# Pointcept/Pointcept

Measured on AMD Instinct MI355X. Metric: scenes/sec (fwd+bwd+optimizer) PTv3 ScanNet-semseg @ ~100k pts, higher is better.
Workload: dtype bf16; 1 GPU; PT-v3m1 base (46.2M params) + seg head + CE + Lovasz, fwd+bwd+AdamW, 8 scenes x 102400 voxels per GPU, patch 1024, 4 orders; global_batch=8, parallelism=dp1, params=46167572, amp=bf16 autocast, points_per_gpu=819200, loss=CrossEntropy(ignore_index=-1) + LovaszSoftmax

## Files before the change

### pointcept_amd/csrc/gemm3.h

```cpp
#pragma once
#include "ptc_common.h"

int ptc_gemm3_launch(int dtype, const void* in, int64_t n_in, const void* w, const float* bias, const int32_t* nbr, int64_t n_out, int kv, int c_in,
                     int c_out, void* out, hipStream_t s, int epi, const void* aux_in, void* aux_out);
bool ptc_gemm3_supported(int dtype, int kv, int c_in, int c_out);

#ifdef PTC_GEMM3_IMPL
#include "mma.h"

#define G3_BN 128
#define G3_BK 64
#ifndef G3_STAGGER
#define G3_STAGGER 0
#endif

__device__ __forceinline__ int g3_lds_row_of_channel(int n) { return 16 * ((n & 15) >> 2) + 4 * (n >> 4) + (n & 3); }
template <typename T> __device__ __forceinline__ uint32_t g3_pack2(float lo, float hi);
template <> __device__ __forceinline__ uint32_t g3_pack2<bf16_t>(float lo, float hi) { return ptc_pack_bf16x2(lo, hi); }
template <> __device__ __forceinline__ uint32_t g3_pack2<f16_t>(float lo, float hi) {
  const _Float16 a = (_Float16)lo, b = (_Float16)hi;
  return (uint32_t)(*reinterpret_cast<const uint16_t*>(&a)) | ((uint32_t)(*reinterpret_cast<const uint16_t*>(&b)) << 16);
}
template <typename T> __device__ __forceinline__ void g3_store16(T* dst, const float (&v)[16]) {
  uint32_t pk[8];
#pragma unroll
  for (int i = 0; i < 8; ++i) pk[i] = g3_pack2<T>(v[2 * i], v[2 * i + 1]);
  reinterpret_cast<uint4*>(dst)[0] = make_uint4(pk[0], pk[1], pk[2], pk[3]);
  reinterpret_cast<uint4*>(dst)[1] = make_uint4(pk[4], pk[5], pk[6], pk[7]);
}

__device__ __forceinline__ int g3_off(int row, int p) { return row * (G3_BK * 2) + ((p ^ ((row >> 1) & 7)) << 4); }

template <typename T, int EPI, int RS>
__global__ void __launch_bounds__(256) PTC_WAVES_PER_EU(2, 2)
gemm3_kernel(const T* __restrict__ in, const T* __restrict__ w, const float* __restrict__ bias, const int32_t* __restrict__ nbr, int64_t n_out,
             int kv, int c_in, int c_out, T* __restrict__ out, const T* __restrict__ aux_in, T* __restrict__ aux_out, uint32_t in_bytes,
             int n_col_tiles, int n_tiles) {
  using M = Mma<T>;
  constexpr int BM = RS * 32;
  constexpr int A_BYTES = BM * G3_BK * 2, STAGE_BYTES = A_BYTES + G3_BN * G3_BK * 2;
  extern __shared__ __attribute__((aligned(16))) unsigned char smem[];
  const __amdgpu_buffer_rsrc_t in_buf = ptc_buf(in, in_bytes);
  const int lane = ptc_lane(), wave = threadIdx.x >> 6;
  const int r = lane & 15, g = lane >> 4;
  const int wm = wave & 1, wn = wave >> 1;

  const int PX = (int)gridDim.x >> 3, px = (int)blockIdx.x >> 3, xcd = (int)blockIdx.x & 7;
  const int tx0 = (int)((int64_t)n_tiles * xcd / 8), tx1 = (int)((int64_t)n_tiles * (xcd + 1) / 8);
  if (tx0 + px >= tx1) return;
  if (G3_STAGGER > 0 && px >= PX / 2) __builtin_amdgcn_s_sleep(G3_STAGGER);
  const int n_my = (tx1 - tx0 - px + PX - 1) / PX;
  const int cpk = c_in / G3_BK, cpt = kv * cpk, total = n_my * cpt;

  const int kp = threadIdx.x & 7, rr = threadIdx.x >> 3;
  int lds_a[RS], lds_w[4];
#pragma unroll
  for (int i = 0; i < RS; ++i) lds_a[i] = g3_off(rr + 32 * i, kp);
#pragma unroll
  for (int i = 0; i < 4; ++i) {
    const int row = rr + 32 * i;
    lds_w[i] = A_BYTES + g3_off((row & 64) + g3_lds_row_of_channel(row & 63), kp);
  }

  int lj = 0, lk = 0, lc = 0;
  int64_t l_row0 = 0;
  int l_n0 = 0;
  uint32_t a_cur[RS];
  int32_t idx_next[RS];
  const T* w_cur[4];
  f32x4 bias_r[4];
  ptc_i32x4 ra0[RS], rw0[4], ra1[RS], rw1[4];
  auto set_tile = [&]() __attribute__((always_inline)) {
    const int t = tx0 + px + lj * PX;
    const int row_tile = t / n_col_tiles;
    l_row0 = (int64_t)row_tile * BM;
    l_n0 = (t - row_tile * n_col_tiles) * G3_BN;
  };
  auto request_idx = [&](int j, int k) __attribute__((always_inline)) {
    const int t = tx0 + px + j * PX;
    const int64_t row0 = (int64_t)(t / n_col_tiles) * BM;
#pragma unroll
    for (int i = 0; i < RS; ++i) {
      const int64_t row = row0 + rr + 32 * i;
      int32_t v = -1;
      if (row < n_out) v = nbr ? nbr[(int64_t)k * n_out + row] : (int32_t)row;
      idx_next[i] = v;
    }
  };
  auto enter_segment = [&]() __attribute__((always_inline)) {
#pragma unroll
    for (int i = 0; i < RS; ++i)
      a_cur[i] = idx_next[i] >= 0 ? ((uint32_t)idx_next[i] * (uint32_t)c_in + (uint32_t)(kp * 8)) * 2u : PTC_BUF_OOB;
#pragma unroll
    for (int i = 0; i < 4; ++i) w_cur[i] = w + ((int64_t)(l_n0 + rr + 32 * i) * kv + lk) * c_in + kp * 8;
  };
  auto issue_chunk = [&](ptc_i32x4 (&ra)[RS], ptc_i32x4 (&rw)[4]) __attribute__((always_inline)) {
    const int c0 = lc * G3_BK;
#pragma unroll
    for (int i = 0; i < RS; ++i)
      ra[i] = __builtin_amdgcn_raw_buffer_load_b128(in_buf, (int)(a_cur[i] == PTC_BUF_OOB ? PTC_BUF_OOB : a_cur[i] + (uint32_t)c0 * 2u), 0, 0);
#pragma unroll
    for (int i = 0; i < 4; ++i) rw[i] = *reinterpret_cast<const ptc_i32x4*>(w_cur[i] + c0);
  };
  auto request_bias = [&]() __attribute__((always_inline)) {
#pragma unroll
    for (int t = 0; t < 4; ++t) {
      bias_r[t] = (f32x4){0.f, 0.f, 0.f, 0.f};
      if (bias) bias_r[t] = *reinterpret_cast<const f32x4*>(bias + l_n0 + wn * 64 + 16 * g + 4 * t);
    }
  };
  auto request_following = [&]() __attribute__((always_inline)) {
    if (lk + 1 < kv) request_idx(lj, lk + 1);
    else if (lj + 1 < n_my) request_idx(lj + 1, 0);
  };
  auto store_chunk = [&](int st, const ptc_i32x4 (&ra)[RS], const ptc_i32x4 (&rw)[4]) __attribute__((always_inline)) {
    unsigned char* base = smem + st * STAGE_BYTES;
#pragma unroll
    for (int i = 0; i < RS; ++i) *reinterpret_cast<ptc_i32x4*>(base + lds_a[i]) = ra[i];
#pragma unroll
    for (int i = 0; i < 4; ++i) *reinterpret_cast<ptc_i32x4*>(base + lds_w[i]) = rw[i];
  };
  auto advance = [&]() __attribute__((always_inline)) {
    if (++lc == cpk) {
      lc = 0;
      if (++lk == kv) { lk = 0; ++lj; }
    }
  };

  int64_t p_row0 = 0;
  int p_n0 = 0;
  auto fetch = [&](ptc_i32x4 (&ra)[RS], ptc_i32x4 (&rw)[4], bool live) __attribute__((always_inline)) {
    const bool seg_start = live && lc == 0, tile_start = seg_start && lk == 0;
    if (tile_start) { set_tile(); p_row0 = l_row0; p_n0 = l_n0; }
    if (seg_start) enter_segment();
    if (tile_start) request_bias();
    if (seg_start) request_following();
    issue_chunk(ra, rw);
    if (live) advance();
  };

  request_idx(0, 0);
  fetch(ra0, rw0, true);
  int64_t c_row0 = p_row0;
  int c_n0 = p_n0;
  int crem = 0;
  fetch(ra1, rw1, true);
  store_chunk(0, ra0, rw0);
  __syncthreads();

  f32x4 acc[RS][4];
  auto half = [&](int it, ptc_i32x4 (&raL)[RS], ptc_i32x4 (&rwL)[4], const ptc_i32x4 (&raS)[RS], const ptc_i32x4 (&rwS)[4]) __attribute__((always_inline)) {
    if (crem == 0) {
#pragma unroll
      for (int t = 0; t < 4; ++t)
#pragma unroll
        for (int s = 0; s < RS; ++s) acc[s][t] = bias_r[t];
    }
    fetch(raL, rwL, it + 2 < total);
    const unsigned char* As = smem + (it & 1) * STAGE_BYTES;
    const unsigned char* Ws = As + A_BYTES;
#pragma unroll
    for (int ks = 0; ks < G3_BK / 32; ++ks) {
      typename M::frag fw[4], fa[RS];
#pragma unroll
      for (int t = 0; t < 4; ++t) fw[t] = *reinterpret_cast<const typename M::frag*>(Ws + g3_off(wn * 64 + t * 16 + r, ks * 4 + g));
#pragma unroll
      for (int s = 0; s < RS; ++s) fa[s] = *reinterpret_cast<const typename M::frag*>(As + g3_off(wm * (RS * 16) + s * 16 + r, ks * 4 + g));
#pragma unroll
      for (int s = 0; s < RS; ++s)
#pragma unroll
        for (int t = 0; t < 4; ++t) acc[s][t] = M::mma(fw[t], fa[s], acc[s][t]);
    }
    if (crem == cpt - 1) {
#pragma unroll
      for (int s = 0; s < RS; ++s) {
        const int64_t row = c_row0 + wm * (RS * 16) + s * 16 + r;
        if (row >= n_out) continue;
        const int64_t off = row * c_out + c_n0 + wn * 64 + 16 * g;
        float v[16];
#pragma unroll
        for (int t = 0; t < 4; ++t)
#pragma unroll
          for (int e = 0; e < 4; ++e) v[4 * t + e] = acc[s][t][e];
        if constexpr (EPI == 2) {
          T hv[16];
          *reinterpret_cast<uint4*>(hv) = reinterpret_cast<const uint4*>(aux_in + off)[0];
          *reinterpret_cast<uint4*>(hv + 8) = reinterpret_cast<const uint4*>(aux_in + off)[1];
#pragma unroll
          for (int i = 0; i < 16; ++i) v[i] *= ptc_gelu_grad(ptc_to_float(hv[i]));
        }
        g3_store16<T>(out + off, v);
        if constexpr (EPI == 1) {
          float u[16];
#pragma unroll
          for (int i = 0; i < 16; ++i) u[i] = ptc_gelu(ptc_to_float(ptc_from_float<T>(v[i])));
          g3_store16<T>(aux_out + off, u);
        }
      }
      crem = 0;
      c_row0 = p_row0;
      c_n0 = p_n0;
    } else {
      ++crem;
    }
    if (it + 1 < total) store_chunk((it + 1) & 1, raS, rwS);
    __syncthreads();
  };
  int it = 0;
#pragma unroll 1
  for (; it + 1 < total; it += 2) {
    half(it, ra0, rw0, ra1, rw1);
    half(it + 1, ra1, rw1, ra0, rw0);
  }
  if (it < total) half(it, ra0, rw0, ra1, rw1);
}

static inline bool gemm3_enabled() {
  static const bool on = [] { const char* e = getenv("PTC_GEMM3"); return !(e && e[0] == '0'); }();
  return on;
}
bool ptc_gemm3_supported(int dtype, int kv, int c_in, int c_out) {
  return gemm3_enabled() && dtype != PTC_F32 && kv >= 1 && kv <= 4 && c_in >= 128 && c_in % G3_BK == 0 && c_out % G3_BN == 0;
}

template <typename T>
static int launch_gemm3(const void* in, int64_t n_in, const void* w, const float* bias, const int32_t* nbr, int64_t n_out, int kv, int c_in, int c_out,
                        void* out, hipStream_t s, int epi, const void* aux_in, void* aux_out) {
  const int n_col = c_out / G3_BN;
  const bool small = ptc_cdiv(n_out, 128) * n_col < 512;
  const int bm = small ? 64 : 128;
  const int64_t n_tiles = ptc_cdiv(n_out, bm) * n_col;
  if (n_tiles > 0x7fffffffll) { ptc_set_error("gemm3: %lld tiles", (long long)n_tiles); return PTC_EUNSUPPORTED; }
  int64_t wgs = (n_tiles + 7) & ~(int64_t)7;
  if (wgs > 512) wgs = 512;
  const dim3 grid((unsigned)wgs);
  const uint32_t in_bytes = (uint32_t)((uint64_t)n_in * c_in * sizeof(T));
#define G3_LAUNCH_RS(EE, RR)                                                                                                           \
  {                                                                                                                                    \
    auto kern = gemm3_kernel<T, EE, RR>;                                                                                               \
    const int lds = 2 * (RR * 32 + G3_BN) * G3_BK * 2;                                                                                 \
    PTC_HIP(hipFuncSetAttribute(reinterpret_cast<const void*>(kern), hipFuncAttributeMaxDynamicSharedMemorySize, lds));                \
    hipLaunchKernelGGL(kern, grid, dim3(256), lds, s, (const T*)in, (const T*)w, bias, nbr, n_out, kv, c_in, c_out, (T*)out,           \
                       (const T*)aux_in, (T*)aux_out, in_bytes, n_col, (int)n_tiles);                                                  \
  }
#define G3_LAUNCH(EE) { if (small) G3_LAUNCH_RS(EE, 2) else G3_LAUNCH_RS(EE, 4) }
  if (epi == 1) G3_LAUNCH(1) else if (epi == 2) G3_LAUNCH(2) else G3_LAUNCH(0)
#undef G3_LAUNCH
#undef G3_LAUNCH_RS
  PTC_CHECK_LAUNCH("gemm3_kernel");
  return PTC_OK;
}

int ptc_gemm3_launch(int dtype, const void* in, int64_t n_in, const void* w, const float* bias, const int32_t* nbr, int64_t n_out, int kv, int c_in,
                     int c_out, void* out, hipStream_t s, int epi, const void* aux_in, void* aux_out) {
  if (dtype == PTC_BF16) return launch_gemm3<bf16_t>(in, n_in, w, bias, nbr, n_out, kv, c_in, c_out, out, s, epi, aux_in, aux_out);
  return launch_gemm3<f16_t>(in, n_in, w, bias, nbr, n_out, kv, c_in, c_out, out, s, epi, aux_in, aux_out);
}
#endif
```

Before: 231.0 scenes/s.

## Add A-resident gathered GEMM kernel for kv=1 with streamed weight ring

Adds gemm3r_kernel, used by default for kv==1 and c_in<=256. It loads a 64-row gathered A tile into LDS once through direct global-to-LDS DMA, then streams weight chunks through a 3-stage ring across all output column tiles, so the gathered input is not re-read for each column tile. Jobs are split by row tile and column group so there are enough workgroups. It also generalizes the XCD-aware tile walk and adds an env override for the grid size. The cost is inline asm with manual waitcnt/barrier handling, which is fragile, and more LDS per block, which can lower occupancy.

```diff
diff --git a/pointcept_amd/csrc/gemm3.h b/pointcept_amd/csrc/gemm3.h
--- a/pointcept_amd/csrc/gemm3.h
+++ b/pointcept_amd/csrc/gemm3.h
@@ -30,6 +30,84 @@
 }
 
 __device__ __forceinline__ int g3_off(int row, int p) { return row * (G3_BK * 2) + ((p ^ ((row >> 1) & 7)) << 4); }
+
+template <typename T, int EPI, int RS>
+__device__ __forceinline__ void g3_epilogue(const f32x4 (&acc)[RS][4], int64_t row0, int n0, int64_t n_out, int c_out, int wm, int wn, int r, int g,
+                                            T* __restrict__ out, const T* __restrict__ aux_in, T* __restrict__ aux_out) {
+#pragma unroll
+  for (int s = 0; s < RS; ++s) {
+    const int64_t row = row0 + wm * (RS * 16) + s * 16 + r;
+    if (row >= n_out) continue;
+    const int64_t off = row * c_out + n0 + wn * 64 + 16 * g;
+    float v[16];
+#pragma unroll
+    for (int t = 0; t < 4; ++t)
+#pragma unroll
+      for (int e = 0; e < 4; ++e) v[4 * t + e] = acc[s][t][e];
+    if constexpr (EPI == 2) {
+      T hv[16];
+      *reinterpret_cast<uint4*>(hv) = reinterpret_cast<const uint4*>(aux_in + off)[0];
+      *reinterpret_cast<uint4*>(hv + 8) = reinterpret_cast<const uint4*>(aux_in + off)[1];
+#pragma unroll
+      for (int i = 0; i < 16; ++i) v[i] *= ptc_gelu_grad(ptc_to_float(hv[i]));
+    }
+    g3_store16<T>(out + off, v);
+    if constexpr (EPI == 1) {
+      float u[16];
+#pragma unroll
+      for (int i = 0; i < 16; ++i) u[i] = ptc_gelu(ptc_to_float(ptc_from_float<T>(v[i])));
+      g3_store16<T>(aux_out + off, u);
+    }
+  }
+}
+
+struct G3Walk { int first, stride, count; };
+__device__ __forceinline__ G3Walk g3_walk(int n_items) {
+  const int G = (int)gridDim.x, nx = G < 8 ? G : 8;
+  const int x = (int)blockIdx.x % nx, px = (int)blockIdx.x / nx, PX = (G - x + nx - 1) / nx;
+  const int i0 = (int)((int64_t)n_items * x / nx), i1 = (int)((int64_t)n_items * (x + 1) / nx);
+  G3Walk wk;
+  wk.first = i0 + px;
+  wk.stride = PX;
+  wk.count = i0 + px < i1 ? (i1 - i0 - px + PX - 1) / PX : 0;
+  return wk;
+}
+
+#define G3_WAIT_LGKM0 0xC07F
+#define G3_WAIT_VM(n) (0x0F70 | ((n) & 15) | (((n) >> 4) << 14))
+#ifdef __HIPCC__
+__device__ __forceinline__ void g3_dma16(const void* g, uint32_t lds_dst) {
+  unsigned keep;
+  asm volatile("s_mov_b32 %0, m0\n\ts_mov_b32 m0, %2\n\ts_nop 0\n\tglobal_load_lds_dwordx4 %1, off\n\ts_mov_b32 m0, %0"
+               : "=&s"(keep) : "v"(g), "s"(lds_dst) : "memory");
+}
+__device__ __forceinline__ void g3_dma16s(const void* sbase, uint32_t voff, uint32_t lds_dst) {
+  unsigned keep;
+  asm volatile("s_mov_b32 %0, m0\n\ts_mov_b32 m0, %3\n\ts_nop 0\n\tglobal_load_lds_dwordx4 %1, %2\n\ts_mov_b32 m0, %0"
+               : "=&s"(keep) : "v"(voff), "s"(sbase), "s"(lds_dst) : "memory");
+}
+__device__ __forceinline__ uint32_t g3_lds_addr(const void* p) { return (uint32_t)(uintptr_t)(const __attribute__((address_space(3))) void*)p; }
+typedef float g3_f32x16 __attribute__((ext_vector_type(16), aligned(4)));
+__device__ __forceinline__ void g3_bias16(const float* p, int g, float (&bv)[16]) {
+  const __attribute__((address_space(4))) g3_f32x16* q = (const __attribute__((address_space(4))) g3_f32x16*)(uintptr_t)p;
+#pragma unroll
+  for (int gg = 0; gg < 4; ++gg) {
+    const g3_f32x16 x = q[gg];
+#pragma unroll
+    for (int i = 0; i < 16; ++i) bv[i] = g == gg ? x[i] : bv[i];
+  }
+}
+#else
+__device__ __forceinline__ void g3_dma16(const void* g, uint32_t lds_dst) { emu_global_load_lds(g, smem + lds_dst, 16); }
+__device__ __forceinline__ void g3_dma16s(const void* sbase, uint32_t voff, uint32_t lds_dst) {
+  emu_global_load_lds(reinterpret_cast<const unsigned char*>(sbase) + voff, smem + lds_dst, 16);
+}
+__device__ __forceinline__ uint32_t g3_lds_addr(const void* p) { return (uint32_t)((const unsigned char*)p - smem); }
+__device__ __forceinline__ void g3_bias16(const float* p, int g, float (&bv)[16]) {
+  for (int i = 0; i < 16; ++i) bv[i] = p[16 * g + i];
+}
+#endif
+static __device__ __attribute__((aligned(16))) const unsigned char g3_zero16[16] = {0};
 
 template <typename T, int EPI, int RS>
 __global__ void __launch_bounds__(256) PTC_WAVES_PER_EU(2, 2)
@@ -45,11 +123,10 @@
   const int r = lane & 15, g = lane >> 4;
   const int wm = wave & 1, wn = wave >> 1;
 
-  const int PX = (int)gridDim.x >> 3, px = (int)blockIdx.x >> 3, xcd = (int)blockIdx.x & 7;
-  const int tx0 = (int)((int64_t)n_tiles * xcd / 8), tx1 = (int)((int64_t)n_tiles * (xcd + 1) / 8);
-  if (tx0 + px >= tx1) return;
-  if (G3_STAGGER > 0 && px >= PX / 2) __builtin_amdgcn_s_sleep(G3_STAGGER);
-  const int n_my = (tx1 - tx0 - px + PX - 1) / PX;
+  const G3Walk wk = g3_walk(n_tiles);
+  if (wk.count == 0) return;
+  const int PX = wk.stride, tx0 = 0, px = wk.first, n_my = wk.count;
+  if (G3_STAGGER > 0 && (int)blockIdx.x >= (int)gridDim.x / 2) __builtin_amdgcn_s_sleep(G3_STAGGER);
   const int cpk = c_in / G3_BK, cpt = kv * cpk, total = n_my * cpt;
 
   const int kp = threadIdx.x & 7, rr = threadIdx.x >> 3;
@@ -172,31 +249,7 @@
         for (int t = 0; t < 4; ++t) acc[s][t] = M::mma(fw[t], fa[s], acc[s][t]);
     }
     if (crem == cpt - 1) {
-#pragma unroll
-      for (int s = 0; s < RS; ++s) {
-        const int64_t row = c_row0 + wm * (RS * 16) + s * 16 + r;
-        if (row >= n_out) continue;
-        const int64_t off = row * c_out + c_n0 + wn * 64 + 16 * g;
-        float v[16];
-#pragma unroll
-        for (int t = 0; t < 4; ++t)
-#pragma unroll
-          for (int e = 0; e < 4; ++e) v[4 * t + e] = acc[s][t][e];
-        if constexpr (EPI == 2) {
-          T hv[16];
-          *reinterpret_cast<uint4*>(hv) = reinterpret_cast<const uint4*>(aux_in + off)[0];
-          *reinterpret_cast<uint4*>(hv + 8) = reinterpret_cast<const uint4*>(aux_in + off)[1];
-#pragma unroll
-          for (int i = 0; i < 16; ++i) v[i] *= ptc_gelu_grad(ptc_to_float(hv[i]));
-        }
-        g3_store16<T>(out + off, v);
-        if constexpr (EPI == 1) {
-          float u[16];
-#pragma unroll
-          for (int i = 0; i < 16; ++i) u[i] = ptc_gelu(ptc_to_float(ptc_from_float<T>(v[i])));
-          g3_store16<T>(aux_out + off, u);
-        }
-      }
+      g3_epilogue<T, EPI, RS>(acc, c_row0, c_n0, n_out, c_out, wm, wn, r, g, out, aux_in, aux_out);
       crem = 0;
       c_row0 = p_row0;
       c_n0 = p_n0;
@@ -215,6 +268,127 @@
   if (it < total) half(it, ra0, rw0, ra1, rw1);
 }
 
+#define G3R_MAX_CIN 256
+#define G3R_NS 3
+template <typename T, int EPI>
+__global__ void __launch_bounds__(256) PTC_WAVES_PER_EU(2, 2)
+gemm3r_kernel(const T* __restrict__ in, const T* __restrict__ w, const float* __restrict__ bias, const int32_t* __restrict__ nbr, int64_t n_out,
+              int c_in, int c_out, T* __restrict__ out, const T* __restrict__ aux_in, T* __restrict__ aux_out, int col_split, int n_jobs) {
+  using M = Mma<T>;
+  constexpr int RS = 2, BM = 64, A_CHUNK = BM * G3_BK * 2, W_STAGE = G3_BN * G3_BK * 2;
+  extern __shared__ __attribute__((aligned(16))) unsigned char smem[];
+  const int lane = ptc_lane(), wave = __builtin_amdgcn_readfirstlane((int)(threadIdx.x >> 6));
+  const int r = lane & 15, g = lane >> 4;
+  const int wm = wave & 1, wn = wave >> 1;
+  const int cpk = c_in / G3_BK, cols = (c_out / G3_BN) / col_split, total = cols * cpk;
+  const G3Walk wk = g3_walk(n_jobs);
+  if (wk.count == 0) return;
+  const uint32_t lds0 = (uint32_t)__builtin_amdgcn_readfirstlane((int)g3_lds_addr(smem));
+  const uint32_t ring0 = lds0 + (uint32_t)(cpk * A_CHUNK);
+  const unsigned char* ringp = smem + cpk * A_CHUNK;
+
+  const int dl = lane >> 3, kp = (lane & 7) ^ ((4 * wave + (lane >> 4)) & 7);
+  uint32_t w_off[4];
+#pragma unroll
+  for (int i = 0; i < 4; ++i) {
+    const int L = 8 * wave + 32 * i + dl;
+    const int ch = (L & 64) + 16 * ((L >> 2) & 3) + 4 * ((L >> 4) & 3) + (L & 3);
+    w_off[i] = ((uint32_t)ch * (uint32_t)c_in + (uint32_t)(kp * 8)) * 2u;
+  }
+  int32_t idx_next[RS];
+  auto request_idx = [&](int job) __attribute__((always_inline)) {
+    const int64_t row0 = (int64_t)(job / col_split) * BM;
+#pragma unroll
+    for (int i = 0; i < RS; ++i) {
+      const int64_t row = row0 + 8 * wave + 32 * i + dl;
+      int32_t v = -1;
+      if (row < n_out) v = nbr ? nbr[row] : (int32_t)row;
+      idx_next[i] = v;
+    }
+  };
+  request_idx(wk.first);
+
+#pragma unroll 1
+  for (int j = 0; j < wk.count; ++j) {
+    const int job = wk.first + j * wk.stride;
+    const int row_tile = job / col_split;
+    const int64_t row0 = (int64_t)row_tile * BM;
+    const int nbase = (job - row_tile * col_split) * cols * G3_BN;
+
+    {
+      const unsigned char* a_src[RS];
+      int a_step[RS];
+#pragma unroll
+      for (int i = 0; i < RS; ++i) {
+        const bool present = idx_next[i] >= 0;
+        a_src[i] = present ? reinterpret_cast<const unsigned char*>(in) + ((int64_t)idx_next[i] * c_in + kp * 8) * 2 : g3_zero16;
+        a_step[i] = present ? G3_BK * 2 : 0;
+      }
+      for (int cc = 0; cc < cpk; ++cc)
+#pragma unroll
+        for (int i = 0; i < RS; ++i)
+          g3_dma16(a_src[i] + cc * a_step[i], lds0 + (uint32_t)(cc * A_CHUNK + (8 * wave + 32 * i) * (G3_BK * 2)));
+    }
+    if (j + 1 < wk.count) request_idx(job + wk.stride);
+
+    int lt = 0, lc = 0, ls = 0;
+    auto issue_w = [&]() __attribute__((always_inline)) {
+      const uint32_t base = ((uint32_t)(nbase + lt * G3_BN) * (uint32_t)c_in + (uint32_t)(lc * G3_BK)) * 2u;
+#pragma unroll
+      for (int i = 0; i < 4; ++i) g3_dma16s(w, base + w_off[i], ring0 + (uint32_t)(ls * W_STAGE + (8 * wave + 32 * i) * (G3_BK * 2)));
+      if (++lc == cpk) { lc = 0; ++lt; }
+      if (++ls == G3R_NS) ls = 0;
+    };
+    issue_w();
+    issue_w();
+    __builtin_amdgcn_s_waitcnt(G3_WAIT_VM(4) & G3_WAIT_LGKM0);
+    __builtin_amdgcn_s_barrier();
+
+    f32x4 acc[RS][4];
+    int cc = 0, ct = 0, st = 0;
+#pragma unroll 1
+    for (int q = 0; q < total; ++q) {
+      if (cc == 0) {
+        float bv[16];
+#pragma unroll
+        for (int i = 0; i < 16; ++i) bv[i] = 0.f;
+        if (bias) g3_bias16(bias + __builtin_amdgcn_readfirstlane(nbase + ct * G3_BN + wn * 64), g, bv);
+#pragma unroll
+        for (int t = 0; t < 4; ++t)
+#pragma unroll
+          for (int s = 0; s < RS; ++s) acc[s][t] = (f32x4){bv[4 * t], bv[4 * t + 1], bv[4 * t + 2], bv[4 * t + 3]};
+      }
+      if (q + 2 < total) issue_w();
+      const unsigned char* As = smem + cc * A_CHUNK;
+      const unsigned char* Ws = ringp + st * W_STAGE;
+#pragma unroll
+      for (int ks = 0; ks < G3_BK / 32; ++ks) {
+        typename M::frag fw[4], fa[RS];
+#pragma unroll
+        for (int t = 0; t < 4; ++t) fw[t] = *reinterpret_cast<const typename M::frag*>(Ws + g3_off(wn * 64 + t * 16 + r, ks * 4 + g));
+#pragma unroll
+        for (int s = 0; s < RS; ++s) fa[s] = *reinterpret_cast<const typename M::frag*>(As + g3_off(wm * (RS * 16) + s * 16 + r, ks * 4 + g));
+#pragma unroll
+        for (int s = 0; s < RS; ++s)
+#pragma unroll
+          for (int t = 0; t < 4; ++t) acc[s][t] = M::mma(fw[t], fa[s], acc[s][t]);
+      }
+      if (cc == cpk - 1) {
+        g3_epilogue<T, EPI, RS>(acc, row0, nbase + ct * G3_BN, n_out, c_out, wm, wn, r, g, out, aux_in, aux_out);
+        cc = 0;
+        ++ct;
+      } else {
+        ++cc;
+      }
+      if (++st == G3R_NS) st = 0;
+      if (q + 2 < total) __builtin_amdgcn_s_waitcnt(G3_WAIT_VM(4) & G3_WAIT_LGKM0);
+      else if (q + 1 < total) __builtin_amdgcn_s_waitcnt(G3_WAIT_VM(0) & G3_WAIT_LGKM0);
+      else __builtin_amdgcn_s_waitcnt(G3_WAIT_LGKM0);
+      __builtin_amdgcn_s_barrier();
+    }
+  }
+}
+
 static inline bool gemm3_enabled() {
   static const bool on = [] { const char* e = getenv("PTC_GEMM3"); return !(e && e[0] == '0'); }();
   return on;
@@ -223,9 +397,47 @@
   return gemm3_enabled() && dtype != PTC_F32 && kv >= 1 && kv <= 4 && c_in >= 128 && c_in % G3_BK == 0 && c_out % G3_BN == 0;
 }
 
+static inline int64_t gemm3_cap_wgs(int64_t wgs) {
+  if (const char* e = getenv("PTC_GEMM3_WGS")) { const int v = atoi(e); if (v > 0 && v < wgs) wgs = v; }
+  return wgs;
+}
+static inline bool gemm3_resident(int kv, int c_in) {
+  static const bool on = [] { const char* e = getenv("PTC_GEMM3_RESIDENT"); return !(e && e[0] == '0'); }();
+  return on && kv == 1 && c_in <= G3R_MAX_CIN;
+}
+
+template <typename T>
+static int launch_gemm3r(const void* in, const void* w, const float* bias, const int32_t* nbr, int64_t n_out, int c_in, int c_out, void* out,
+                         hipStream_t s, int epi, const void* aux_in, void* aux_out) {
+  const int n_col = c_out / G3_BN;
+  const int64_t row_tiles = ptc_cdiv(n_out, 64);
+  int split = n_col;
+  for (int d = 1; d <= n_col; ++d)
+    if (n_col % d == 0 && row_tiles * d >= 512) { split = d; break; }
+  const int64_t n_jobs = row_tiles * split;
+  if (n_jobs > 0x7fffffffll || (uint64_t)c_out * c_in * sizeof(T) > 0xffffffffull) { ptc_set_error("gemm3: %lld jobs", (long long)n_jobs); return PTC_EUNSUPPORTED; }
+  if (n_jobs == 0) return PTC_OK;
+  int64_t wgs = (n_jobs + 7) & ~(int64_t)7;
+  if (wgs > 512) wgs = 512;
+  const dim3 grid((unsigned)gemm3_cap_wgs(wgs));
+  const int lds = 64 * c_in * 2 + G3R_NS * G3_BN * G3_BK * 2;
+#define G3R_LAUNCH(EE)                                                                                                                 \
+  {                                                                                                                                    \
+    auto kern = gemm3r_kernel<T, EE>;                                                                                                  \
+    PTC_HIP(hipFuncSetAttribute(reinterpret_cast<const void*>(kern), hipFuncAttributeMaxDynamicSharedMemorySize, lds));                \
+    hipLaunchKernelGGL(kern, grid, dim3(256), lds, s, (const T*)in, (const T*)w, bias, nbr, n_out, c_in, c_out, (T*)out,               \
+                       (const T*)aux_in, (T*)aux_out, split, (int)n_jobs);                                                             \
+  }
+  if (epi == 1) G3R_LAUNCH(1) else if (epi == 2) G3R_LAUNCH(2) else G3R_LAUNCH(0)
+#undef G3R_LAUNCH
+  PTC_CHECK_LAUNCH("gemm3r_kernel");
+  return PTC_OK;
+}
+
 template <typename T>
 static int launch_gemm3(const void* in, int64_t n_in, const void* w, const float* bias, const int32_t* nbr, int64_t n_out, int kv, int c_in, int c_out,
                         void* out, hipStream_t s, int epi, const void* aux_in, void* aux_out) {
+  if (gemm3_resident(kv, c_in)) return launch_gemm3r<T>(in, w, bias, nbr, n_out, c_in, c_out, out, s, epi, aux_in, aux_out);
   const int n_col = c_out / G3_BN;
   const bool small = ptc_cdiv(n_out, 128) * n_col < 512;
   const int bm = small ? 64 : 128;
@@ -233,7 +445,7 @@
   if (n_tiles > 0x7fffffffll) { ptc_set_error("gemm3: %lld tiles", (long long)n_tiles); return PTC_EUNSUPPORTED; }
   int64_t wgs = (n_tiles + 7) & ~(int64_t)7;
   if (wgs > 512) wgs = 512;
-  const dim3 grid((unsigned)wgs);
+  const dim3 grid((unsigned)gemm3_cap_wgs(wgs));
   const uint32_t in_bytes = (uint32_t)((uint64_t)n_in * c_in * sizeof(T));
 #define G3_LAUNCH_RS(EE, RR)                                                                                                           \
   {                                                                                                                                    \
```

Result: no change. 229.7 scenes/s (-0.5%).
